# wenbowen123/iros20-6d-pose-tracking

Measured on AMD Instinct MI355X. Metric: RGB-D pair inferences/sec (176x176), higher is better.
Workload: dtype f32; 1 GPU; configs[1]: batch=64 synthetic 176x176 RGB-D pairs per GPU, random-init Se3TrackNet (reference state_dict surface), stage=full; pairs_per_gpu=64, global_batch=64, stage=full, frames=resident in HBM

## Files before the change

### iros20-6d-pose-tracking_amd/csrc/api.cpp

```cpp
#include <cmath>
#include <thread>
#include <cstdio>
#include <cstdlib>
#include <chrono>
#include <cstring>
#include <map>
#include <mutex>
#include <string>
#include <vector>

#include "se3tn_internal.h"
#include "weights.h"

using namespace se3tn;

static thread_local std::string g_err;
static int fail(int code, const std::string& msg) {
  g_err = msg;
  return code;
}
static int hipfail(hipError_t e, const char* what) {
  g_err = std::string(what) + ": " + hipGetErrorString(e);
  return (int)e;
}
// ... 7 lines not shown

struct GraphKey {
  const void *A, *B, *trans, *rot, *poseA, *poseB, *blob;
  int n, layout, prec, wino_min_batch, wino_tile, keep, wino64, wino64_fill;
  int small_kernels, splitk_fused, wino_fuse, gemmp, tail_parts;
  double tn, rn;
  bool operator==(const GraphKey& o) const { return std::memcmp(this, &o, sizeof(GraphKey)) == 0; }
};
struct GraphEntry {
  GraphKey key;
  hipGraphExec_t exec = nullptr;
  bool fast = false;
  const float* head_final = nullptr;
};

struct se3tn_ctx {
  int device = -1, max_batch = 0;
  TensorMap tensors;
  std::vector<float> packed;
  float* blob_owned = nullptr;
  const float* blob = nullptr;
  BlobLayout L;
  float *inA = nullptr, *inB = nullptr;
  float* stem = nullptr;
  float *pool = nullptr, *t64 = nullptr, *q64 = nullptr;
  float *ab = nullptr, *ab_t = nullptr;
  float *head = nullptr, *head_t = nullptr;
  float* head_f = nullptr;
  const float* head_final = nullptr;
  float* logits = nullptr;
  float* fcpart = nullptr;
  bool keep_intermediates = false;
  int auto_tile_override[2] = {0, 0};
  int trunk_kernel = 1;
  int gemmp = -1;
  bool wino_fuse = true;
  float* part = nullptr;
  int* splitk_sem = nullptr;
  int tail_parts_ch = 16;
  bool tail_parts = true;
  bool small_kernels = true;
  bool splitk_fused = false;
  size_t part_bytes = 0;
  int wino_min_batch = SE3TN_WINOGRAD_DEFAULT_MIN_BATCH;
  int wino_tile = SE3TN_WINOGRAD_DEFAULT_TILE;
  int wino_tile_derived = 0;
  float* wino_u[4] = {nullptr, nullptr, nullptr, nullptr};
  float* wino_u6[4] = {nullptr, nullptr, nullptr, nullptr};
  const float* wino6_blob = nullptr;
  float *wino_v = nullptr, *wino_m = nullptr;
  const float* wino_blob = nullptr;
  int wino64_min_batch = SE3TN_TRUNK_WINOGRAD_DEFAULT_MIN_BATCH;
  int wino64_min_fill = SE3TN_TRUNK_WINOGRAD_DEFAULT_MIN_FILL;
  int num_cus = 256;
  float* wino64_u[4] = {nullptr, nullptr, nullptr, nullptr};
  const float* wino64_blob = nullptr;
  SplitLayout SL;
  float* split_w = nullptr;
  const float* split_blob = nullptr;
  float* wino_us[4] = {nullptr, nullptr, nullptr, nullptr};
  float* wino_usc[4] = {nullptr, nullptr, nullptr, nullptr};
  const float* wino_us_blob = nullptr;
  int wino_us_tile = 0;
  int prec = SE3TN_PREC_F32;
  int offset_rule = SE3TN_OFFSET_RULE_NUMPY1;
  int raster_sub_bits = 4;
  uint8_t* trk_host = nullptr; uint8_t* trk_dev = nullptr; size_t trk_bytes = 0;
// ... 183 lines not shown
  c->fd_buf = nullptr; c->fd_pixels = 0;
  HIPCHK(hipMalloc((void**)&c->fd_buf, (3 * px + 2 + 4098 + 2) * sizeof(float)));
  c->fd_pixels = px;
  return SE3TN_OK;
}
static int reserve_zbuf(se3tn_ctx* c, size_t px) {
  if (px <= c->zbuf_px) return SE3TN_OK;
  HIPCHK(hipDeviceSynchronize());
  if (c->zbuf) HIPCHK(hipFree(c->zbuf));
  c->zbuf = nullptr; c->zbuf_px = 0;
  HIPCHK(hipMalloc((void**)&c->zbuf, sizeof(unsigned long long) * px));
  c->zbuf_px = px;
  return SE3TN_OK;
}
static bool stream_is_capturing(hipStream_t st) {
  hipStreamCaptureStatus cs = hipStreamCaptureStatusNone;
  return hipStreamIsCapturing(st, &cs) == hipSuccess && cs != hipStreamCaptureStatusNone;
}

extern "C" {

const char* se3tn_version(void) { return "se3tracknet-gfx950 0.5.0 (blob v7)"; }
const char* se3tn_last_error(void) { return g_err.c_str(); }

int se3tn_create(int device, int max_batch, se3tn_ctx** out) {
  if (!out || max_batch < 1) return fail(SE3TN_E_ARG, "se3tn_create: bad argument");
  se3tn_ctx* c = new se3tn_ctx();
  c->device = device;
  c->max_batch = max_batch;
  c->L = blob_layout();
  c->SL = split_layout();
  if (const char* e = std::getenv("SE3TN_WINOGRAD_AUTO_TILE_AB2")) c->auto_tile_override[0] = (std::atoi(e) == 4 || std::atoi(e) == 6) ? std::atoi(e) : 0;
  if (const char* e = std::getenv("SE3TN_WINOGRAD_AUTO_TILE_HEADS")) c->auto_tile_override[1] = (std::atoi(e) == 4 || std::atoi(e) == 6) ? std::atoi(e) : 0;
  if (const char* e = std::getenv("SE3TN_TRUNK_KERNEL")) c->trunk_kernel = std::atoi(e) == 2 ? 2 : 1;
  if (const char* e = std::getenv("SE3TN_WINO_GEMMP")) c->gemmp = std::atoi(e) != 0 ? 1 : 0;
  if (const char* e = std::getenv("SE3TN_WINOGRAD_FUSE")) c->wino_fuse = std::atoi(e) != 0;
  if (const char* e = std::getenv("SE3TN_TRUNK_WINOGRAD")) c->wino64_min_batch = std::atoi(e);
  if (const char* e = std::getenv("SE3TN_TRUNK_WINOGRAD_FILL")) c->wino64_min_fill = std::atoi(e);
  for (int i = 0; i < 8; ++i) { c->mean[i] = 0.0; c->stdv[i] = 1.0; }
  if (device >= 0) {
    hipDeviceProp_t prop;
    hipError_t e = hipGetDeviceProperties(&prop, device);
    if (e != hipSuccess) { delete c; return hipfail(e, "hipGetDeviceProperties"); }
    if (std::strncmp(prop.gcnArchName, "gfx950", 6) != 0) {
      std::string a = prop.gcnArchName;
      delete c;
      return fail(SE3TN_E_DEVICE, "device is " + a + ", this library is built for gfx950 only");
    }
    if (prop.multiProcessorCount > 0) c->num_cus = prop.multiProcessorCount;
    e = hipSetDevice(device);
    if (e != hipSuccess) { delete c; return hipfail(e, "hipSetDevice"); }
    const size_t mb = (size_t)max_batch;
    auto padded = [&](int s, int ch) { return (mb * (s + 2) * (s + 2) + PAD_SLACK_PX) * ch; };
    struct { float** p; size_t words; bool zero; } bufs[] = {
        {&c->inA, (mb * IN_P + IN_SLACK_ROWS) * IN_P * 4, true},
        {&c->inB, (mb * IN_P + IN_SLACK_ROWS) * IN_P * 4, true},
        {&c->stem, mb * S1 * S1 * 128, false}, {&c->pool, padded(S2, 128), true},
        {&c->t64, padded(S2, 128), true},      {&c->q64, padded(S2, 128), true},
        {&c->ab, padded(S3, 256), true},       {&c->ab_t, padded(S3, 256), true},
        {&c->head, padded(S4, 1024), true},    {&c->head_t, padded(S4, 1024), true},
        {&c->head_f, padded(S4, 1024), true},
        {&c->logits, mb * 6, true},           {&c->fcpart, mb * 192, true}};
    for (auto& b : bufs) {
      e = hipMalloc((void**)b.p, b.words * sizeof(float));
      if (e != hipSuccess) { se3tn_destroy(c); return hipfail(e, "hipMalloc(workspace)"); }
      if (b.zero) e = hipMemset(*b.p, 0, b.words * sizeof(float));
      if (e != hipSuccess) { se3tn_destroy(c); return hipfail(e, "hipMemset(workspace)"); }
// ... 1426 lines not shown
```

### iros20-6d-pose-tracking_amd/csrc/wino64_fused.hip

```cpp
#include "mfma_common.h"

#ifndef W64_KNOCKOUT
#define W64_KNOCKOUT 0
#endif

namespace se3tn {

namespace {
constexpr int W64_TILES = 11;
constexpr int W64_PATCH = 2 * W64_TILES + 2;
constexpr int W64_PATCH_FLOATS = W64_PATCH * W64_PATCH * 32;
constexpr int W64_V_FLOATS = 128 * 32, W64_U_FLOATS = 64 * 32;
constexpr int W64_UBUFS = 2;
constexpr int W64_LDS_FLOATS = W64_PATCH_FLOATS + 2 * W64_V_FLOATS + W64_UBUFS * W64_U_FLOATS;
constexpr int W64_YLDS_FLOATS = W64_TILES * W64_TILES * (4 * 64 + 4);
constexpr size_t W64_LDS_BYTES = sizeof(float) * (W64_YLDS_FLOATS > W64_LDS_FLOATS ? W64_YLDS_FLOATS : W64_LDS_FLOATS);
}

__device__ __forceinline__ void bt_row(int i, int& r0, int& r1, float& c0, float& c1) {
  r0 = i == 0 ? 0 : 1;
  r1 = i == 3 ? 3 : 2;
  c0 = i == 2 ? -1.f : 1.f;
  c1 = (i == 0 || i == 3) ? -1.f : 1.f;
}
__device__ __forceinline__ void at_col(int i, float& a0, float& a1) {
  a0 = i == 3 ? 0.f : 1.f;
  a1 = i == 0 ? 0.f : (i == 1 ? 1.f : -1.f);
}

template <bool NA, bool NB>
__device__ __forceinline__ float add_pm(const float a, const float b) {
  float r;
  if constexpr (!NA && !NB) asm volatile("v_add_f32 %0, %1, %2" : "=v"(r) : "v"(a), "v"(b));
  else if constexpr (NA && !NB) asm volatile("v_sub_f32 %0, %2, %1" : "=v"(r) : "v"(a), "v"(b));
  else if constexpr (!NA && NB) asm volatile("v_sub_f32 %0, %1, %2" : "=v"(r) : "v"(a), "v"(b));
  else asm volatile("v_sub_f32 %0, -%1, %2" : "=v"(r) : "v"(a), "v"(b));
  return r;
}
template <int K>
__device__ __forceinline__ void acc_pm(float& y, const float m) {
  if constexpr (K > 0) asm volatile("v_add_f32 %0, %0, %1" : "+v"(y) : "v"(m));
  else if constexpr (K < 0) asm volatile("v_sub_f32 %0, %0, %1" : "+v"(y) : "v"(m));
}
struct W64Tab {
  static constexpr int bt_r0(int i) { return i == 0 ? 0 : 1; }
  static constexpr int bt_r1(int i) { return i == 3 ? 3 : 2; }
  static constexpr bool bt_n0(int i) { return i == 2; }
  static constexpr bool bt_n1(int i) { return i == 0 || i == 3; }
  static constexpr int at(int y, int i) { return y == 0 ? (i == 3 ? 0 : 1) : (i == 0 ? 0 : (i == 1 ? 1 : -1)); }
  static constexpr int off(int r, int s) { return (r * W64_PATCH + (s >> 1) + 12 * (s & 1)) * 32; }
};

struct Wino64Args {
  const float* in;
  const float* U;
  const float* bias;
  const float* res;
  float* out;
  int in_ld, res_ld, out_ld;
  int in_gs, res_gs, out_gs, bias_gs;
  long long u_gs;
  int n, groups;
};

template <int EPI>
__global__ __launch_bounds__(512) void wino64_fused_kernel(const Wino64Args a) {
  extern __shared__ __attribute__((aligned(16))) float smem[];
  float* patch = smem;
  float* Vb = smem + W64_PATCH_FLOATS;
  float* Ub = Vb + 2 * W64_V_FLOATS;

  const int tid = threadIdx.x, lane = tid & 63;
  const int wid = __builtin_amdgcn_readfirstlane(tid >> 6);
  const int rb = wid >> 1, cbk = wid & 1;
  const int l31 = lane & 31, hh = lane >> 5;

  const int g = blockIdx.x % a.groups, rest = blockIdx.x / a.groups;
  const int quad = rest & 3, img = rest >> 2;
  const int y0 = (quad >> 1) * 2 * W64_TILES, x0 = (quad & 1) * 2 * W64_TILES;
  constexpr int HP = 46;
  const float* __restrict__ in = a.in + (size_t)g * a.in_gs + ((size_t)(img * HP + y0) * HP + x0) * a.in_ld;
  const float* __restrict__ Ug = a.U + (size_t)g * a.u_gs;
  const unsigned lds0 = __builtin_amdgcn_readfirstlane(lds_addr_of(smem));

  const int ur = tid >> 3;
  const unsigned uvoff = (unsigned)((ur * 32 + (((tid & 7) ^ ((ur >> 1) & 7)) << 2)) * 4);

#define W64_ISSUE_PATCH(CH)                                                                                     \
  {                                                                                                            \
    const float* pb_ = in + (CH) * 32;                                                                          \
    _Pragma("unroll") for (int j_ = 0; j_ < 9; ++j_) {                                \
      const int id_ = tid + 512 * j_, px_ = id_ >> 3, py_ = px_ / W64_PATCH, pxx_ = px_ - py_ * W64_PATCH;      \
      const int xs_ = pxx_ < 12 ? 2 * pxx_ : 2 * pxx_ - 23;           \
      glds16<0>(pb_, (unsigned)(((py_ * HP + xs_) * a.in_ld + (id_ & 7) * 4) * 4),                              \
                lds0 + (unsigned)((wid * 64 + 512 * j_) * 16));                                                 \
    }                                                                                                          \
  }
#define W64_ISSUE_U(CH, F, BUFI)                                                                                \
  glds16<0>(Ug + (size_t)((CH) * 16 + (F)) * W64_U_FLOATS, uvoff,                                              \
            lds0 + (unsigned)((W64_PATCH_FLOATS + 2 * W64_V_FLOATS + (BUFI) * W64_U_FLOATS + wid * 256) * 4));

  int tpix[2], tdst[2];
#pragma unroll
  for (int j = 0; j < 2; ++j) {
    const int tt = (tid + 512 * j) >> 3, tcb = tid & 7;
    const int ttr = tt < W64_TILES * W64_TILES ? tt : W64_TILES * W64_TILES - 1;
    const int tty = ttr / W64_TILES, ttx = ttr - tty * W64_TILES;
    tpix[j] = ((2 * tty) * W64_PATCH + ttx) * 32 + tcb * 4;
    tdst[j] = tt * 32 + ((tcb ^ ((tt >> 1) & 7)) << 2);
  }
#define W64_BT(F)                                                                                               \
  int r0_, r1_, s0_, s1_;                                                                                      \
  float cr0_, cr1_, cs0_, cs1_;                                                                                \
  bt_row((F) >> 2, r0_, r1_, cr0_, cr1_);                                                                      \
  bt_row((F) & 3, s0_, s1_, cs0_, cs1_);                                                                       \
  const int q0_ = (s0_ >> 1) + 12 * (s0_ & 1), q1_ = (s1_ >> 1) + 12 * (s1_ & 1);              \
  const int o00_ = (r0_ * W64_PATCH + q0_) * 32, o01_ = (r0_ * W64_PATCH + q1_) * 32;                          \
  const int o10_ = (r1_ * W64_PATCH + q0_) * 32, o11_ = (r1_ * W64_PATCH + q1_) * 32;                          \
  const float c00_ = cr0_ * cs0_, c01_ = cr0_ * cs1_, c10_ = cr1_ * cs0_, c11_ = cr1_ * cs1_;
#define W64_TR_LOAD(D)                                                                                          \
  _Pragma("unroll") for (int j_ = 0; j_ < 2; ++j_) {                                                            \
    D[j_][0] = *reinterpret_cast<const float4*>(patch + tpix[j_] + o00_);                                       \
    D[j_][1] = *reinterpret_cast<const float4*>(patch + tpix[j_] + o01_);                                       \
    D[j_][2] = *reinterpret_cast<const float4*>(patch + tpix[j_] + o10_);                                       \
    D[j_][3] = *reinterpret_cast<const float4*>(patch + tpix[j_] + o11_);                                       \
  }
#define W64_TR_STORE(D, VBUF)                                                                                   \
  _Pragma("unroll") for (int j_ = 0; j_ < 2; ++j_) {                                                            \
    float4 v_;                                                                                                 \
    v_.x = c00_ * D[j_][0].x + c01_ * D[j_][1].x + c10_ * D[j_][2].x + c11_ * D[j_][3].x;                       \
    v_.y = c00_ * D[j_][0].y + c01_ * D[j_][1].y + c10_ * D[j_][2].y + c11_ * D[j_][3].y;                       \
    v_.z = c00_ * D[j_][0].z + c01_ * D[j_][1].z + c10_ * D[j_][2].z + c11_ * D[j_][3].z;                       \
    v_.w = c00_ * D[j_][0].w + c01_ * D[j_][1].w + c10_ * D[j_][2].w + c11_ * D[j_][3].w;                       \
    *reinterpret_cast<float4*>(Vb + (VBUF) * W64_V_FLOATS + tdst[j_]) = v_;                                     \
  }
#define W64_TRANSFORM(F, VBUF)                                                                                  \
  {                                                                                                            \
    W64_BT(F)                                                                                                  \
    float4 d_[2][4];                                                                                           \
    W64_TR_LOAD(d_)                                                                                            \
    W64_TR_STORE(d_, VBUF)                                                                                     \
  }

  const int X = (l31 >> 1) & 7;
  const int lo = (hh ^ (X & 1)) * 4, xk = X >> 1;
  const int fo0 = ((0 ^ xk) << 3) + lo, fo1 = ((1 ^ xk) << 3) + lo, fo2 = ((2 ^ xk) << 3) + lo, fo3 = ((3 ^ xk) << 3) + lo;

  float Y[16][4];
#pragma unroll
  for (int e = 0; e < 16; ++e)
#pragma unroll
    for (int o = 0; o < 4; ++o) Y[e][o] = 0.f;

  W64_ISSUE_PATCH(0)
  W64_ISSUE_U(0, 0, 0)
  wait_dma_and_barrier();
  W64_TRANSFORM(0, 0)
  __syncthreads();

  f32x16 accA, accB;
#pragma unroll
  for (int e = 0; e < 16; ++e) accB[e] = 0.f;
  const f32x16 zero16 = {0.f, 0.f, 0.f, 0.f, 0.f, 0.f, 0.f, 0.f, 0.f, 0.f, 0.f, 0.f, 0.f, 0.f, 0.f, 0.f};
#define W64_FOLD(PREV, F)                                                                                       \
  {                                                                                                            \
    float ay0_, ay1_, ax0_, ax1_;                                                                              \
    at_col((F) >> 2, ay0_, ay1_);                                                                              \
    at_col((F) & 3, ax0_, ax1_);                                                                               \
    const float k00_ = ay0_ * ax0_, k01_ = ay0_ * ax1_, k10_ = ay1_ * ax0_, k11_ = ay1_ * ax1_;                \
    _Pragma("unroll") for (int e_ = 0; e_ < 16; ++e_) {                                                        \
      const float m_ = PREV[e_];                                                                               \
      Y[e_][0] += k00_ * m_; Y[e_][1] += k01_ * m_; Y[e_][2] += k10_ * m_; Y[e_][3] += k11_ * m_;              \
    }                                                                                                          \
  }
#define W64_MFMA(ACC)                                                                                        \
  ACC = q_ == 0 ? __builtin_amdgcn_mfma_f32_32x32x2f32(wv_[0], pv_[0], zero16, 0, 0, 0)                         \
                : __builtin_amdgcn_mfma_f32_32x32x2f32(wv_[q_], pv_[q_], ACC, 0, 0, 0);
#define W64_STEP(F, ACC, PREV)                                                                                  \
  {                                                                                                            \
    constexpr int f_ = (F), buf = f_ & 1, fn_ = (f_ + 1) & 15, fp_ = (f_ + 15) & 15;                            \
    const bool last_ = ch == 1 && f_ == 15;                                                                    \
    if (!last_) W64_ISSUE_U(f_ == 15 ? 1 : ch, fn_, buf ^ 1)                                                    \
    if (f_ == 15 && ch == 0) W64_ISSUE_PATCH(1)  \
    {                                                                                                          \
      const float* pP = Vb + buf * W64_V_FLOATS + (rb * 32 + l31) * 32;                                        \
      const float* pW = Ub + buf * W64_U_FLOATS + (cbk * 32 + l31) * 32;                                       \
      float pv_[16], wv_[16];                                                                                  \
      float d_[2][4][4], v_[2][4];                                       \
      *reinterpret_cast<float4*>(pv_ + 0) = *reinterpret_cast<const float4*>(pP + fo0);                         \
      *reinterpret_cast<float4*>(wv_ + 0) = *reinterpret_cast<const float4*>(pW + fo0);                         \
      *reinterpret_cast<float4*>(pv_ + 4) = *reinterpret_cast<const float4*>(pP + fo1);                         \
      *reinterpret_cast<float4*>(wv_ + 4) = *reinterpret_cast<const float4*>(pW + fo1);                         \
      *reinterpret_cast<float4*>(pv_ + 8) = *reinterpret_cast<const float4*>(pP + fo2);                         \
      *reinterpret_cast<float4*>(wv_ + 8) = *reinterpret_cast<const float4*>(pW + fo2);                         \
      *reinterpret_cast<float4*>(pv_ + 12) = *reinterpret_cast<const float4*>(pP + fo3);                        \
      *reinterpret_cast<float4*>(wv_ + 12) = *reinterpret_cast<const float4*>(pW + fo3);                        \
                              \
       \
      constexpr int i_ = fn_ >> 2, j_ = fn_ & 3;                                                               \
      constexpr int oo_[4] = {W64Tab::off(W64Tab::bt_r0(i_), W64Tab::bt_r0(j_)), W64Tab::off(W64Tab::bt_r0(i_), W64Tab::bt_r1(j_)), \
                              W64Tab::off(W64Tab::bt_r1(i_), W64Tab::bt_r0(j_)), W64Tab::off(W64Tab::bt_r1(i_), W64Tab::bt_r1(j_))}; \
      constexpr bool nn_[4] = {W64Tab::bt_n0(i_) != W64Tab::bt_n0(j_), W64Tab::bt_n0(i_) != W64Tab::bt_n1(j_),  \
                               W64Tab::bt_n1(i_) != W64Tab::bt_n0(j_), W64Tab::bt_n1(i_) != W64Tab::bt_n1(j_)}; \
      _Pragma("unroll") for (int t_ = 0; t_ < 2; ++t_)                                                          \
        _Pragma("unroll") for (int w_ = 0; w_ < 4; ++w_) {                                                      \
          if (W64_KNOCKOUT & 1) *reinterpret_cast<float4*>(d_[t_][w_]) = make_float4(1.f, 2.f, 3.f, 4.f);  \
          else *reinterpret_cast<float4*>(d_[t_][w_]) = *reinterpret_cast<const float4*>(patch + tpix[t_] + oo_[w_]); \
        }                                                                                                      \
      constexpr int pi_ = fp_ >> 2, pj_ = fp_ & 3;    \
      __builtin_amdgcn_sched_barrier(0);                                                                       \
      _Pragma("unroll") for (int q_ = 0; q_ < 16; ++q_) {                                                       \
        W64_MFMA(ACC)                                                                                          \
        __builtin_amdgcn_sched_barrier(0);                                                                     \
        if (q_ < 8) {                             \
          _Pragma("unroll") for (int e_ = 2 * q_; e_ < 2 * q_ + 2; ++e_) {                                      \
            const float m_ = PREV[e_];                                                                         \
            acc_pm<W64Tab::at(0, pi_) * W64Tab::at(0, pj_)>(Y[e_][0], m_);                                     \
            acc_pm<W64Tab::at(0, pi_) * W64Tab::at(1, pj_)>(Y[e_][1], m_);                                     \
            acc_pm<W64Tab::at(1, pi_) * W64Tab::at(0, pj_)>(Y[e_][2], m_);                                     \
            acc_pm<W64Tab::at(1, pi_) * W64Tab::at(1, pj_)>(Y[e_][3], m_);                                     \
          }                                                                                                    \
        } else {               \
          const int t_ = (q_ - 8) >> 2, x_ = (q_ - 8) & 3;                                                     \
          v_[t_][x_] = add_pm<false, false>(add_pm<nn_[0], nn_[1]>(d_[t_][0][x_], d_[t_][1][x_]),              \
                                            add_pm<nn_[2], nn_[3]>(d_[t_][2][x_], d_[t_][3][x_]));             \
        }                                                                                                      \
        __builtin_amdgcn_sched_barrier(0);                                                                     \
      }                                                                                                        \
      *reinterpret_cast<float4*>(Vb + (buf ^ 1) * W64_V_FLOATS + tdst[0]) = *reinterpret_cast<float4*>(v_[0]); \
      *reinterpret_cast<float4*>(Vb + (buf ^ 1) * W64_V_FLOATS + tdst[1]) = *reinterpret_cast<float4*>(v_[1]); \
    }                                                                                                          \
    if (!last_) wait_dma_and_barrier();                                                                        \
    if (f_ == 15 && ch == 0) {  \
      W64_TRANSFORM(0, 0)                                                                                      \
      __syncthreads();                                                                                         \
    }                                                                                                          \
  }
  for (int ch = 0; ch < 2; ++ch) {
    W64_STEP(0, accA, accB) W64_STEP(1, accB, accA) W64_STEP(2, accA, accB) W64_STEP(3, accB, accA)
    W64_STEP(4, accA, accB) W64_STEP(5, accB, accA) W64_STEP(6, accA, accB) W64_STEP(7, accB, accA)
    W64_STEP(8, accA, accB) W64_STEP(9, accB, accA) W64_STEP(10, accA, accB) W64_STEP(11, accB, accA)
    W64_STEP(12, accA, accB) W64_STEP(13, accB, accA) W64_STEP(14, accA, accB) W64_STEP(15, accB, accA)
  }
  W64_FOLD(accB, 15)
#undef W64_STEP
#undef W64_MFMA
#undef W64_FOLD
#undef W64_ISSUE_PATCH
#undef W64_ISSUE_U
#undef W64_TRANSFORM
#undef W64_TR_LOAD
#undef W64_TR_STORE
#undef W64_BT

  constexpr int YS = 4 * 64 + 4;
  __syncthreads();
  {
    const int t = rb * 32 + l31;
    if (t < W64_TILES * W64_TILES) {
#pragma unroll
      for (int o = 0; o < 4; ++o)
#pragma unroll
        for (int q = 0; q < 4; ++q)
          *reinterpret_cast<float4*>(smem + t * YS + o * 64 + cbk * 32 + q * 8 + hh * 4) =
              make_float4(Y[4 * q + 0][o], Y[4 * q + 1][o], Y[4 * q + 2][o], Y[4 * q + 3][o]);
    }
  }
  const float* __restrict__ bias = a.bias + (size_t)g * a.bias_gs;
  const float* __restrict__ res = (EPI == 1) ? a.res + (size_t)g * a.res_gs : nullptr;
  float* __restrict__ out = a.out + (size_t)g * a.out_gs;
  const int c4 = (tid & 15) * 4;
  __syncthreads();
  const float4 b = *reinterpret_cast<const float4*>(bias + c4);
#pragma unroll 4
  for (int k = 0; k < 16; ++k) {
    const int p = (k * 512 + tid) >> 4;
    const int t = p >> 2, o = p & 3;
    if (t < W64_TILES * W64_TILES) {
      const int ty = t / W64_TILES, tx = t - ty * W64_TILES;
      const int oy = y0 + 2 * ty + (o >> 1) + 1, ox = x0 + 2 * tx + (o & 1) + 1;
      const size_t pix = (size_t)(img * HP + oy) * HP + ox;
      float4 v = *reinterpret_cast<const float4*>(smem + t * YS + o * 64 + c4);
      v.x += b.x; v.y += b.y; v.z += b.z; v.w += b.w;
      if (EPI == 1) {
        const float4 r = *reinterpret_cast<const float4*>(res + pix * a.res_ld + c4);
        v.x += r.x; v.y += r.y; v.z += r.z; v.w += r.w;
      }
      v.x = fmaxf(v.x, 0.f); v.y = fmaxf(v.y, 0.f); v.z = fmaxf(v.z, 0.f); v.w = fmaxf(v.w, 0.f);
      *reinterpret_cast<float4*>(out + pix * a.out_ld + c4) = v;
    }
  }
}

#ifndef SE3TN_TRUNK_REGV
#define SE3TN_TRUNK_REGV 0
#endif
#if SE3TN_TRUNK_REGV
typedef float f32x4 __attribute__((ext_vector_type(4)));

template <int EPI>
__global__ __launch_bounds__(512) void wino64_regv_kernel(const Wino64Args a) {
  extern __shared__ __attribute__((aligned(16))) float smem[];
  const int tid = threadIdx.x, lane = tid & 63;
  const int wid = __builtin_amdgcn_readfirstlane(tid >> 6);
  const int r16 = lane & 15, jq = lane >> 4;

  const int g = blockIdx.x % a.groups, rest = blockIdx.x / a.groups;
  const int quad = rest & 3, img = rest >> 2;
  const int y0 = (quad >> 1) * 2 * W64_TILES, x0 = (quad & 1) * 2 * W64_TILES;
  constexpr int HP = 46;
  const float* __restrict__ in = a.in + (size_t)g * a.in_gs + ((size_t)(img * HP + y0) * HP + x0) * a.in_ld;
  const float* __restrict__ Ug = a.U + (size_t)g * a.u_gs;
  const unsigned lds0 = __builtin_amdgcn_readfirstlane(lds_addr_of(smem));

#define W64R_ISSUE_PATCH(CH)                                                                                    \
  {                                                                                                            \
    const float* pb_ = in + (CH) * 32;                                                                          \
    _Pragma("unroll") for (int j_ = 0; j_ < 9; ++j_) {                                                          \
      const int id_ = tid + 512 * j_, px_ = id_ >> 3, py_ = px_ / W64_PATCH, lc_ = px_ - py_ * W64_PATCH;       \
      const int xs_ = lc_ < 12 ? 2 * lc_ : 2 * lc_ - 23;                                                        \
      glds16<0>(pb_, (unsigned)(((py_ * HP + xs_) * a.in_ld + (((id_ & 7) ^ (lc_ & 7)) << 2)) * 4),             \
                lds0 + (unsigned)(((CH) * W64_PATCH_FLOATS) * 4 + (wid * 64 + 512 * j_) * 16));                 \
    }                                                                                                          \
  }
// ... 126 lines not shown
  const float4 bq = *reinterpret_cast<const float4*>(bias + c4);
#pragma unroll 4
  for (int k = 0; k < 16; ++k) {
    const int p = (k * 512 + tid) >> 4;
    const int t = p >> 2, o = p & 3;
    if (t < W64_TILES * W64_TILES) {
      const int ty = t / W64_TILES, tx = t - ty * W64_TILES;
      const int oy = y0 + 2 * ty + (o >> 1) + 1, ox = x0 + 2 * tx + (o & 1) + 1;
      const size_t pix = (size_t)(img * HP + oy) * HP + ox;
      float4 v = *reinterpret_cast<const float4*>(smem + t * YS + o * 64 + c4);
      v.x += bq.x; v.y += bq.y; v.z += bq.z; v.w += bq.w;
      if (EPI == 1) {
        const float4 r = *reinterpret_cast<const float4*>(res + pix * a.res_ld + c4);
        v.x += r.x; v.y += r.y; v.z += r.z; v.w += r.w;
      }
      v.x = fmaxf(v.x, 0.f); v.y = fmaxf(v.y, 0.f); v.z = fmaxf(v.z, 0.f); v.w = fmaxf(v.w, 0.f);
      *reinterpret_cast<float4*>(out + pix * a.out_ld + c4) = v;
    }
  }
}

#endif

hipError_t launch_wino64(const float* in, int in_ld, int in_gs, const float* U, long long u_gs, const float* bias, int bias_gs,
                         const float* res, int res_ld, int res_gs, float* out, int out_ld, int out_gs, int n, int groups, int epi,
                         int variant, hipStream_t st) {
  Wino64Args a{};
  a.in = in; a.U = U; a.bias = bias; a.res = res; a.out = out;
  a.in_ld = in_ld; a.res_ld = res_ld; a.out_ld = out_ld;
  a.in_gs = in_gs; a.res_gs = res_gs; a.out_gs = out_gs; a.bias_gs = bias_gs; a.u_gs = u_gs;
  a.n = n; a.groups = groups;
  constexpr size_t lds2 = sizeof(float) * 2 * W64_PATCH_FLOATS;
  static_assert(lds2 >= sizeof(float) * W64_YLDS_FLOATS, "the epilogue staging must fit the patch buffers");
  static PerDeviceOnce attr[4];
#if !SE3TN_TRUNK_REGV
  variant = 1;
#endif
  const void* kern = epi == 1 ? reinterpret_cast<const void*>(wino64_fused_kernel<1>) : reinterpret_cast<const void*>(wino64_fused_kernel<0>);
#if SE3TN_TRUNK_REGV
  if (variant == 2) kern = epi == 1 ? reinterpret_cast<const void*>(wino64_regv_kernel<1>) : reinterpret_cast<const void*>(wino64_regv_kernel<0>);
#endif
  const size_t lds = variant == 2 ? lds2 : W64_LDS_BYTES;
  bool* done = attr[(variant == 2 ? 2 : 0) + (epi == 1 ? 1 : 0)].current();
  if (!done || !*done) {
    hipError_t e = hipFuncSetAttribute(kern, hipFuncAttributeMaxDynamicSharedMemorySize, (int)lds);
    if (e != hipSuccess) return e;
    if (done) *done = true;
  }
  const dim3 grid(n * 4 * groups);
#if SE3TN_TRUNK_REGV
  if (variant == 2) {
    if (epi == 1) hipLaunchKernelGGL(wino64_regv_kernel<1>, grid, dim3(512), lds, st, a);
    else hipLaunchKernelGGL(wino64_regv_kernel<0>, grid, dim3(512), lds, st, a);
    return hipGetLastError();
  }
#endif
  if (epi == 1) hipLaunchKernelGGL(wino64_fused_kernel<1>, grid, dim3(512), lds, st, a);
  else hipLaunchKernelGGL(wino64_fused_kernel<0>, grid, dim3(512), lds, st, a);
  return hipGetLastError();
}

}
```

Measured before the change: 41960 pairs/s.

## Split trunk Winograd patch loads into half-row chunks interleaved across filter steps

Result: no change. 42170 pairs/s, median of 6 (+0.5%).

```diff
diff --git a/iros20-6d-pose-tracking_amd/csrc/api.cpp b/iros20-6d-pose-tracking_amd/csrc/api.cpp
--- a/iros20-6d-pose-tracking_amd/csrc/api.cpp
+++ b/iros20-6d-pose-tracking_amd/csrc/api.cpp
@@ -63,7 +63,7 @@
   float* fcpart = nullptr;
   bool keep_intermediates = false;
   int auto_tile_override[2] = {0, 0};
-  int trunk_kernel = 1;
+  int trunk_kernel = 3;
   int gemmp = -1;
   bool wino_fuse = true;
   float* part = nullptr;
@@ -313,7 +313,7 @@
   c->SL = split_layout();
   if (const char* e = std::getenv("SE3TN_WINOGRAD_AUTO_TILE_AB2")) c->auto_tile_override[0] = (std::atoi(e) == 4 || std::atoi(e) == 6) ? std::atoi(e) : 0;
   if (const char* e = std::getenv("SE3TN_WINOGRAD_AUTO_TILE_HEADS")) c->auto_tile_override[1] = (std::atoi(e) == 4 || std::atoi(e) == 6) ? std::atoi(e) : 0;
-  if (const char* e = std::getenv("SE3TN_TRUNK_KERNEL")) c->trunk_kernel = std::atoi(e) == 2 ? 2 : 1;
+  if (const char* e = std::getenv("SE3TN_TRUNK_KERNEL")) c->trunk_kernel = (std::atoi(e) == 1 || std::atoi(e) == 2) ? std::atoi(e) : 3;
   if (const char* e = std::getenv("SE3TN_WINO_GEMMP")) c->gemmp = std::atoi(e) != 0 ? 1 : 0;
   if (const char* e = std::getenv("SE3TN_WINOGRAD_FUSE")) c->wino_fuse = std::atoi(e) != 0;
   if (const char* e = std::getenv("SE3TN_TRUNK_WINOGRAD")) c->wino64_min_batch = std::atoi(e);
diff --git a/iros20-6d-pose-tracking_amd/csrc/wino64_fused.hip b/iros20-6d-pose-tracking_amd/csrc/wino64_fused.hip
--- a/iros20-6d-pose-tracking_amd/csrc/wino64_fused.hip
+++ b/iros20-6d-pose-tracking_amd/csrc/wino64_fused.hip
@@ -2,6 +2,29 @@
 
 #ifndef W64_KNOCKOUT
 #define W64_KNOCKOUT 0
+#endif
+
+#ifdef SE3TN_W64_TRACE
+#define W64_TRACE_SLOTS 104
+__device__ unsigned long long se3tn_w64_trace[4 * 2 * 8 * W64_TRACE_SLOTS];
+extern "C" int se3tn_debug_w64_trace(void* host_out, size_t bytes, int clear) {
+  if (clear) {
+    void* p = nullptr;
+    if (hipGetSymbolAddress(&p, HIP_SYMBOL(se3tn_w64_trace)) != hipSuccess) return 1;
+    return (int)hipMemset(p, 0, sizeof(se3tn_w64_trace));
+  }
+  return (int)hipMemcpyFromSymbol(host_out, HIP_SYMBOL(se3tn_w64_trace), bytes, 0, hipMemcpyDeviceToHost);
+}
+#define W64_TRACE_SETUP                                                                                          \
+  const bool tr_on_ = lane == 0 && (blockIdx.x == 0 || blockIdx.x == gridDim.x - 1);                              \
+  unsigned long long* tr_ = ::se3tn_w64_trace +                                                                  \
+      ((((a.groups == 2 ? 0 : 2) + EPI) * 2 + (blockIdx.x == 0 ? 0 : 1)) * 8 + wid) * W64_TRACE_SLOTS;
+#define W64_STAMP(I) if (tr_on_) tr_[(I)] = __builtin_amdgcn_s_memtime();
+#define W64_STAMP_RT(I) if (tr_on_) tr_[(I)] = __builtin_amdgcn_s_memrealtime();
+#else
+#define W64_TRACE_SETUP
+#define W64_STAMP(I)
+#define W64_STAMP_RT(I)
 #endif
 
 namespace se3tn {
@@ -63,7 +86,15 @@
   int n, groups;
 };
 
-template <int EPI>
+__device__ __forceinline__ void wait_vm_and_barrier(const int n) {
+  if (n == 0) asm volatile("s_waitcnt vmcnt(0)" ::: "memory");
+  else if (n == 1) asm volatile("s_waitcnt vmcnt(1)" ::: "memory");
+  else if (n == 2) asm volatile("s_waitcnt vmcnt(2)" ::: "memory");
+  else asm volatile("s_waitcnt vmcnt(3)" ::: "memory");
+  __syncthreads();
+}
+
+template <int EPI, bool SPLIT>
 __global__ __launch_bounds__(512) void wino64_fused_kernel(const Wino64Args a) {
   extern __shared__ __attribute__((aligned(16))) float smem[];
   float* patch = smem;
@@ -72,6 +103,9 @@
 
   const int tid = threadIdx.x, lane = tid & 63;
   const int wid = __builtin_amdgcn_readfirstlane(tid >> 6);
+  W64_TRACE_SETUP
+  W64_STAMP_RT(101)
+  W64_STAMP(0)
   const int rb = wid >> 1, cbk = wid & 1;
   const int l31 = lane & 31, hh = lane >> 5;
 
@@ -99,6 +133,16 @@
 #define W64_ISSUE_U(CH, F, BUFI)                                                                                \
   glds16<0>(Ug + (size_t)((CH) * 16 + (F)) * W64_U_FLOATS, uvoff,                                              \
             lds0 + (unsigned)((W64_PATCH_FLOATS + 2 * W64_V_FLOATS + (BUFI) * W64_U_FLOATS + wid * 256) * 4));
+#define W64_ISSUE_HALF(CH, P, J)                                                                                \
+  {                                                                                                            \
+    const int q_ = wid + 8 * (J), hr_ = q_ / 3, py_ = 2 * hr_ + (P), lc0_ = (q_ - 3 * hr_) * 8;                 \
+    const int lc_ = lc0_ + (lane >> 3), xs_ = lc_ < 12 ? 2 * lc_ : 2 * lc_ - 23;                                \
+    glds16<0>(in + (CH) * 32, (unsigned)(((py_ * HP + xs_) * a.in_ld + (lane & 7) * 4) * 4),                    \
+              lds0 + (unsigned)((py_ * W64_PATCH + lc0_) * 32 * 4));                                            \
+  }
+#define W64_ISSUE_HALF_A(CH, P) { W64_ISSUE_HALF(CH, P, 0) W64_ISSUE_HALF(CH, P, 1) if (wid < 4) W64_ISSUE_HALF(CH, P, 4) }
+#define W64_ISSUE_HALF_B(CH, P) { W64_ISSUE_HALF(CH, P, 2) W64_ISSUE_HALF(CH, P, 3) }
+  const int vm_a = wid < 4 ? 3 : 2, vm_b = 2;
 
   int tpix[2], tdst[2];
 #pragma unroll
@@ -152,11 +196,18 @@
 #pragma unroll
     for (int o = 0; o < 4; ++o) Y[e][o] = 0.f;
 
-  W64_ISSUE_PATCH(0)
+  if constexpr (SPLIT) {
+    W64_ISSUE_HALF_A(0, 0)
+    W64_ISSUE_HALF_B(0, 0)
+  } else {
+    W64_ISSUE_PATCH(0)
+  }
   W64_ISSUE_U(0, 0, 0)
   wait_dma_and_barrier();
+  W64_STAMP(1)
   W64_TRANSFORM(0, 0)
   __syncthreads();
+  W64_STAMP(2)
 
   f32x16 accA, accB;
 #pragma unroll
@@ -180,8 +231,17 @@
   {                                                                                                            \
     constexpr int f_ = (F), buf = f_ & 1, fn_ = (f_ + 1) & 15, fp_ = (f_ + 15) & 15;                            \
     const bool last_ = ch == 1 && f_ == 15;                                                                    \
+    W64_STAMP(3 + 3 * (16 * ch + f_))                                                                          \
     if (!last_) W64_ISSUE_U(f_ == 15 ? 1 : ch, fn_, buf ^ 1)                                                    \
-    if (f_ == 15 && ch == 0) W64_ISSUE_PATCH(1)  \
+    int vm_ = 0;    \
+    if constexpr (SPLIT) {                                                                                     \
+      if (f_ == 0 && ch == 0) { W64_ISSUE_HALF_A(0, 1) vm_ = vm_a; }                                           \
+      if (f_ == 1 && ch == 0) { W64_ISSUE_HALF_B(0, 1) vm_ = vm_b; }                                           \
+      if (f_ == 11 && ch == 0) { W64_ISSUE_HALF_A(1, 0) vm_ = vm_a; }   \
+      if (f_ == 12 && ch == 0) { W64_ISSUE_HALF_B(1, 0) vm_ = vm_b; }                                          \
+      if (f_ == 15 && ch == 0) { W64_ISSUE_HALF_A(1, 1) vm_ = vm_a; }   \
+      if (f_ == 0 && ch == 1) { W64_ISSUE_HALF_B(1, 1) vm_ = vm_b; }                                           \
+    } else if (f_ == 15 && ch == 0) W64_ISSUE_PATCH(1)  \
     {                                                                                                          \
       const float* pP = Vb + buf * W64_V_FLOATS + (rb * 32 + l31) * 32;                                        \
       const float* pW = Ub + buf * W64_U_FLOATS + (cbk * 32 + l31) * 32;                                       \
@@ -222,18 +282,28 @@
           }                                                                                                    \
         } else {               \
           const int t_ = (q_ - 8) >> 2, x_ = (q_ - 8) & 3;                                                     \
-          v_[t_][x_] = add_pm<false, false>(add_pm<nn_[0], nn_[1]>(d_[t_][0][x_], d_[t_][1][x_]),              \
-                                            add_pm<nn_[2], nn_[3]>(d_[t_][2][x_], d_[t_][3][x_]));             \
+          if constexpr (SPLIT && fn_ == 0)  \
+            v_[t_][x_] = add_pm<false, nn_[3]>(add_pm<false, nn_[2]>(add_pm<nn_[0], nn_[1]>(d_[t_][0][x_], d_[t_][1][x_]), \
+                                                                     d_[t_][2][x_]), d_[t_][3][x_]);           \
+          else                                                                                                 \
+            v_[t_][x_] = add_pm<false, false>(add_pm<nn_[0], nn_[1]>(d_[t_][0][x_], d_[t_][1][x_]),            \
+                                              add_pm<nn_[2], nn_[3]>(d_[t_][2][x_], d_[t_][3][x_]));           \
         }                                                                                                      \
         __builtin_amdgcn_sched_barrier(0);                                                                     \
       }                                                                                                        \
       *reinterpret_cast<float4*>(Vb + (buf ^ 1) * W64_V_FLOATS + tdst[0]) = *reinterpret_cast<float4*>(v_[0]); \
       *reinterpret_cast<float4*>(Vb + (buf ^ 1) * W64_V_FLOATS + tdst[1]) = *reinterpret_cast<float4*>(v_[1]); \
     }                                                                                                          \
-    if (!last_) wait_dma_and_barrier();                                                                        \
-    if (f_ == 15 && ch == 0) {  \
+    W64_STAMP(4 + 3 * (16 * ch + f_))                                                                          \
+    if (!last_) {                                                                                              \
+      if constexpr (SPLIT) wait_vm_and_barrier(vm_);  \
+      else wait_dma_and_barrier();                                                                             \
+    }                                                                                                          \
+    W64_STAMP(5 + 3 * (16 * ch + f_))                                                                          \
+    if (!SPLIT && f_ == 15 && ch == 0) {  \
       W64_TRANSFORM(0, 0)                                                                                      \
       __syncthreads();                                                                                         \
+      W64_STAMP(103)                                                                                           \
     }                                                                                                          \
   }
   for (int ch = 0; ch < 2; ++ch) {
@@ -243,11 +313,15 @@
     W64_STEP(12, accA, accB) W64_STEP(13, accB, accA) W64_STEP(14, accA, accB) W64_STEP(15, accB, accA)
   }
   W64_FOLD(accB, 15)
+  W64_STAMP(99)
 #undef W64_STEP
 #undef W64_MFMA
 #undef W64_FOLD
 #undef W64_ISSUE_PATCH
 #undef W64_ISSUE_U
+#undef W64_ISSUE_HALF
+#undef W64_ISSUE_HALF_A
+#undef W64_ISSUE_HALF_B
 #undef W64_TRANSFORM
 #undef W64_TR_LOAD
 #undef W64_TR_STORE
@@ -290,6 +364,8 @@
       *reinterpret_cast<float4*>(out + pix * a.out_ld + c4) = v;
     }
   }
+  W64_STAMP(100)
+  W64_STAMP_RT(102)
 }
 
 #ifndef SE3TN_TRUNK_REGV
@@ -482,16 +558,20 @@
   a.n = n; a.groups = groups;
   constexpr size_t lds2 = sizeof(float) * 2 * W64_PATCH_FLOATS;
   static_assert(lds2 >= sizeof(float) * W64_YLDS_FLOATS, "the epilogue staging must fit the patch buffers");
-  static PerDeviceOnce attr[4];
+  static PerDeviceOnce attr[6];
 #if !SE3TN_TRUNK_REGV
-  variant = 1;
-#endif
-  const void* kern = epi == 1 ? reinterpret_cast<const void*>(wino64_fused_kernel<1>) : reinterpret_cast<const void*>(wino64_fused_kernel<0>);
+  if (variant == 2) variant = 3;
+#endif
+  if (variant != 1 && variant != 2) variant = 3;
+  const void* kern = variant == 1 ? (epi == 1 ? reinterpret_cast<const void*>(wino64_fused_kernel<1, false>)
+                                              : reinterpret_cast<const void*>(wino64_fused_kernel<0, false>))
+                                  : (epi == 1 ? reinterpret_cast<const void*>(wino64_fused_kernel<1, true>)
+                                              : reinterpret_cast<const void*>(wino64_fused_kernel<0, true>));
 #if SE3TN_TRUNK_REGV
   if (variant == 2) kern = epi == 1 ? reinterpret_cast<const void*>(wino64_regv_kernel<1>) : reinterpret_cast<const void*>(wino64_regv_kernel<0>);
 #endif
   const size_t lds = variant == 2 ? lds2 : W64_LDS_BYTES;
-  bool* done = attr[(variant == 2 ? 2 : 0) + (epi == 1 ? 1 : 0)].current();
+  bool* done = attr[2 * (variant - 1) + (epi == 1 ? 1 : 0)].current();
   if (!done || !*done) {
     hipError_t e = hipFuncSetAttribute(kern, hipFuncAttributeMaxDynamicSharedMemorySize, (int)lds);
     if (e != hipSuccess) return e;
@@ -505,8 +585,13 @@
     return hipGetLastError();
   }
 #endif
-  if (epi == 1) hipLaunchKernelGGL(wino64_fused_kernel<1>, grid, dim3(512), lds, st, a);
-  else hipLaunchKernelGGL(wino64_fused_kernel<0>, grid, dim3(512), lds, st, a);
+  if (variant == 1) {
+    if (epi == 1) hipLaunchKernelGGL((wino64_fused_kernel<1, false>), grid, dim3(512), lds, st, a);
+    else hipLaunchKernelGGL((wino64_fused_kernel<0, false>), grid, dim3(512), lds, st, a);
+  } else {
+    if (epi == 1) hipLaunchKernelGGL((wino64_fused_kernel<1, true>), grid, dim3(512), lds, st, a);
+    else hipLaunchKernelGGL((wino64_fused_kernel<0, true>), grid, dim3(512), lds, st, a);
+  }
   return hipGetLastError();
 }
 
```

## Reorder Winograd frequencies to accumulate corner terms in MFMA and reuse BT partials

Applied to the files above, without the earlier changes.

Result: no change. 42040 pairs/s before, 42370 pairs/s after, median of 6 (+0.8%).

```diff
diff --git a/iros20-6d-pose-tracking_amd/csrc/wino64_fused.hip b/iros20-6d-pose-tracking_amd/csrc/wino64_fused.hip
--- a/iros20-6d-pose-tracking_amd/csrc/wino64_fused.hip
+++ b/iros20-6d-pose-tracking_amd/csrc/wino64_fused.hip
@@ -17,17 +17,6 @@
 constexpr size_t W64_LDS_BYTES = sizeof(float) * (W64_YLDS_FLOATS > W64_LDS_FLOATS ? W64_YLDS_FLOATS : W64_LDS_FLOATS);
 }
 
-__device__ __forceinline__ void bt_row(int i, int& r0, int& r1, float& c0, float& c1) {
-  r0 = i == 0 ? 0 : 1;
-  r1 = i == 3 ? 3 : 2;
-  c0 = i == 2 ? -1.f : 1.f;
-  c1 = (i == 0 || i == 3) ? -1.f : 1.f;
-}
-__device__ __forceinline__ void at_col(int i, float& a0, float& a1) {
-  a0 = i == 3 ? 0.f : 1.f;
-  a1 = i == 0 ? 0.f : (i == 1 ? 1.f : -1.f);
-}
-
 template <bool NA, bool NB>
 __device__ __forceinline__ float add_pm(const float a, const float b) {
   float r;
@@ -42,6 +31,14 @@
   if constexpr (K > 0) asm volatile("v_add_f32 %0, %0, %1" : "+v"(y) : "v"(m));
   else if constexpr (K < 0) asm volatile("v_sub_f32 %0, %0, %1" : "+v"(y) : "v"(m));
 }
+template <int K>
+__device__ __forceinline__ void acc_pm(f32x16& y, const int e, const float m) {
+  if constexpr (K != 0) {
+    float t = y[e];
+    acc_pm<K>(t, m);
+    y[e] = t;
+  }
+}
 struct W64Tab {
   static constexpr int bt_r0(int i) { return i == 0 ? 0 : 1; }
   static constexpr int bt_r1(int i) { return i == 3 ? 3 : 2; }
@@ -49,6 +46,16 @@
   static constexpr bool bt_n1(int i) { return i == 0 || i == 3; }
   static constexpr int at(int y, int i) { return y == 0 ? (i == 3 ? 0 : 1) : (i == 0 ? 0 : (i == 1 ? 1 : -1)); }
   static constexpr int off(int r, int s) { return (r * W64_PATCH + (s >> 1) + 12 * (s & 1)) * 32; }
+  static constexpr int order(int p) { return p < 4 ? (p == 0 ? 0 : p == 1 ? 3 : p - 1) : p < 8 ? 12 + order(p - 4) : p - 4; }
+  static constexpr bool corner(int f) { return ((f >> 2) == 0 || (f >> 2) == 3) && ((f & 3) == 0 || (f & 3) == 3); }
+  static constexpr int target(int f) { return 2 * ((f >> 2) == 3) + ((f & 3) == 3); }
+  static constexpr int foldk(int f, int o) {
+    return corner(f) ? 0 : at(o >> 1, f >> 2) * at(o & 1, f & 3) * ((o == 1 || o == 2) ? -1 : 1);
+  }
+  static constexpr bool fresh(int f, int s) {
+    return s == 0 || s == 3 || (s == 2 && (f & 3) == 0) ||
+           (s == 1 && ((f & 3) == ((f >> 2) == 0 || (f >> 2) == 3 ? 3 : 1)));
+  }
 };
 
 struct Wino64Args {
@@ -109,79 +116,54 @@
     tpix[j] = ((2 * tty) * W64_PATCH + ttx) * 32 + tcb * 4;
     tdst[j] = tt * 32 + ((tcb ^ ((tt >> 1) & 7)) << 2);
   }
-#define W64_BT(F)                                                                                               \
-  int r0_, r1_, s0_, s1_;                                                                                      \
-  float cr0_, cr1_, cs0_, cs1_;                                                                                \
-  bt_row((F) >> 2, r0_, r1_, cr0_, cr1_);                                                                      \
-  bt_row((F) & 3, s0_, s1_, cs0_, cs1_);                                                                       \
-  const int q0_ = (s0_ >> 1) + 12 * (s0_ & 1), q1_ = (s1_ >> 1) + 12 * (s1_ & 1);              \
-  const int o00_ = (r0_ * W64_PATCH + q0_) * 32, o01_ = (r0_ * W64_PATCH + q1_) * 32;                          \
-  const int o10_ = (r1_ * W64_PATCH + q0_) * 32, o11_ = (r1_ * W64_PATCH + q1_) * 32;                          \
-  const float c00_ = cr0_ * cs0_, c01_ = cr0_ * cs1_, c10_ = cr1_ * cs0_, c11_ = cr1_ * cs1_;
-#define W64_TR_LOAD(D)                                                                                          \
-  _Pragma("unroll") for (int j_ = 0; j_ < 2; ++j_) {                                                            \
-    D[j_][0] = *reinterpret_cast<const float4*>(patch + tpix[j_] + o00_);                                       \
-    D[j_][1] = *reinterpret_cast<const float4*>(patch + tpix[j_] + o01_);                                       \
-    D[j_][2] = *reinterpret_cast<const float4*>(patch + tpix[j_] + o10_);                                       \
-    D[j_][3] = *reinterpret_cast<const float4*>(patch + tpix[j_] + o11_);                                       \
-  }
-#define W64_TR_STORE(D, VBUF)                                                                                   \
-  _Pragma("unroll") for (int j_ = 0; j_ < 2; ++j_) {                                                            \
-    float4 v_;                                                                                                 \
-    v_.x = c00_ * D[j_][0].x + c01_ * D[j_][1].x + c10_ * D[j_][2].x + c11_ * D[j_][3].x;                       \
-    v_.y = c00_ * D[j_][0].y + c01_ * D[j_][1].y + c10_ * D[j_][2].y + c11_ * D[j_][3].y;                       \
-    v_.z = c00_ * D[j_][0].z + c01_ * D[j_][1].z + c10_ * D[j_][2].z + c11_ * D[j_][3].z;                       \
-    v_.w = c00_ * D[j_][0].w + c01_ * D[j_][1].w + c10_ * D[j_][2].w + c11_ * D[j_][3].w;                       \
-    *reinterpret_cast<float4*>(Vb + (VBUF) * W64_V_FLOATS + tdst[j_]) = v_;                                     \
-  }
-#define W64_TRANSFORM(F, VBUF)                                                                                  \
+  float R1[2][4], R2[2][4];
+#define W64_TRANSFORM0()                                                                                        \
   {                                                                                                            \
-    W64_BT(F)                                                                                                  \
-    float4 d_[2][4];                                                                                           \
-    W64_TR_LOAD(d_)                                                                                            \
-    W64_TR_STORE(d_, VBUF)                                                                                     \
+    constexpr int oo_[4] = {W64Tab::off(0, 0), W64Tab::off(2, 0), W64Tab::off(0, 2), W64Tab::off(2, 2)};       \
+    float d_[2][4][4], v_[2][4];                                                                               \
+    _Pragma("unroll") for (int t_ = 0; t_ < 2; ++t_)                                                            \
+      _Pragma("unroll") for (int w_ = 0; w_ < 4; ++w_)                                                          \
+        *reinterpret_cast<float4*>(d_[t_][w_]) = *reinterpret_cast<const float4*>(patch + tpix[t_] + oo_[w_]);  \
+    _Pragma("unroll") for (int t_ = 0; t_ < 2; ++t_)                                                            \
+      _Pragma("unroll") for (int x_ = 0; x_ < 4; ++x_) {                                                        \
+        R2[t_][x_] = add_pm<false, true>(d_[t_][2][x_], d_[t_][3][x_]);                                         \
+        v_[t_][x_] = add_pm<false, true>(add_pm<false, true>(d_[t_][0][x_], d_[t_][1][x_]), R2[t_][x_]);        \
+      }                                                                                                        \
+    *reinterpret_cast<float4*>(Vb + tdst[0]) = *reinterpret_cast<float4*>(v_[0]);                               \
+    *reinterpret_cast<float4*>(Vb + tdst[1]) = *reinterpret_cast<float4*>(v_[1]);                               \
   }
 
   const int X = (l31 >> 1) & 7;
   const int lo = (hh ^ (X & 1)) * 4, xk = X >> 1;
   const int fo0 = ((0 ^ xk) << 3) + lo, fo1 = ((1 ^ xk) << 3) + lo, fo2 = ((2 ^ xk) << 3) + lo, fo3 = ((3 ^ xk) << 3) + lo;
 
-  float Y[16][4];
-#pragma unroll
-  for (int e = 0; e < 16; ++e)
-#pragma unroll
-    for (int o = 0; o < 4; ++o) Y[e][o] = 0.f;
+  f32x16 Yv[4];
+#pragma unroll
+  for (int o = 0; o < 4; ++o)
+#pragma unroll
+    for (int e = 0; e < 16; ++e) Yv[o][e] = 0.f;
 
   W64_ISSUE_PATCH(0)
-  W64_ISSUE_U(0, 0, 0)
+  W64_ISSUE_U(0, W64Tab::order(0), 0)
   wait_dma_and_barrier();
-  W64_TRANSFORM(0, 0)
+  W64_TRANSFORM0()
   __syncthreads();
 
   f32x16 accA, accB;
 #pragma unroll
   for (int e = 0; e < 16; ++e) accB[e] = 0.f;
   const f32x16 zero16 = {0.f, 0.f, 0.f, 0.f, 0.f, 0.f, 0.f, 0.f, 0.f, 0.f, 0.f, 0.f, 0.f, 0.f, 0.f, 0.f};
-#define W64_FOLD(PREV, F)                                                                                       \
+#define W64_MFMA(ACC)                                                                                           \
+  if constexpr (W64Tab::corner(f_)) ACC = __builtin_amdgcn_mfma_f32_32x32x2f32(wv_[q_], pv_[q_], ACC, 0, 0, 0);  \
+  else ACC = q_ == 0 ? __builtin_amdgcn_mfma_f32_32x32x2f32(wv_[0], pv_[0], zero16, 0, 0, 0)                      \
+                     : __builtin_amdgcn_mfma_f32_32x32x2f32(wv_[q_], pv_[q_], ACC, 0, 0, 0);
+#define W64_STEP(P, ACC, PREV)                                                                                  \
   {                                                                                                            \
-    float ay0_, ay1_, ax0_, ax1_;                                                                              \
-    at_col((F) >> 2, ay0_, ay1_);                                                                              \
-    at_col((F) & 3, ax0_, ax1_);                                                                               \
-    const float k00_ = ay0_ * ax0_, k01_ = ay0_ * ax1_, k10_ = ay1_ * ax0_, k11_ = ay1_ * ax1_;                \
-    _Pragma("unroll") for (int e_ = 0; e_ < 16; ++e_) {                                                        \
-      const float m_ = PREV[e_];                                                                               \
-      Y[e_][0] += k00_ * m_; Y[e_][1] += k01_ * m_; Y[e_][2] += k10_ * m_; Y[e_][3] += k11_ * m_;              \
-    }                                                                                                          \
-  }
-#define W64_MFMA(ACC)                                                                                        \
-  ACC = q_ == 0 ? __builtin_amdgcn_mfma_f32_32x32x2f32(wv_[0], pv_[0], zero16, 0, 0, 0)                         \
-                : __builtin_amdgcn_mfma_f32_32x32x2f32(wv_[q_], pv_[q_], ACC, 0, 0, 0);
-#define W64_STEP(F, ACC, PREV)                                                                                  \
-  {                                                                                                            \
-    constexpr int f_ = (F), buf = f_ & 1, fn_ = (f_ + 1) & 15, fp_ = (f_ + 15) & 15;                            \
-    const bool last_ = ch == 1 && f_ == 15;                                                                    \
-    if (!last_) W64_ISSUE_U(f_ == 15 ? 1 : ch, fn_, buf ^ 1)                                                    \
-    if (f_ == 15 && ch == 0) W64_ISSUE_PATCH(1)  \
+    constexpr int p_ = (P), buf = p_ & 1;                                                                      \
+    constexpr int f_ = W64Tab::order(p_), fn_ = W64Tab::order((p_ + 1) & 15), fp_ = W64Tab::order((p_ + 15) & 15); \
+    const bool last_ = ch == 1 && p_ == 15;                                                                    \
+    if (!last_) W64_ISSUE_U(p_ == 15 ? 1 : ch, fn_, buf ^ 1)                                                    \
+    if (p_ == 15 && ch == 0) W64_ISSUE_PATCH(1)  \
     {                                                                                                          \
       const float* pP = Vb + buf * W64_V_FLOATS + (rb * 32 + l31) * 32;                                        \
       const float* pW = Ub + buf * W64_U_FLOATS + (cbk * 32 + l31) * 32;                                       \
@@ -195,35 +177,46 @@
       *reinterpret_cast<float4*>(wv_ + 8) = *reinterpret_cast<const float4*>(pW + fo2);                         \
       *reinterpret_cast<float4*>(pv_ + 12) = *reinterpret_cast<const float4*>(pP + fo3);                        \
       *reinterpret_cast<float4*>(wv_ + 12) = *reinterpret_cast<const float4*>(pW + fo3);                        \
-                              \
        \
-      constexpr int i_ = fn_ >> 2, j_ = fn_ & 3;                                                               \
-      constexpr int oo_[4] = {W64Tab::off(W64Tab::bt_r0(i_), W64Tab::bt_r0(j_)), W64Tab::off(W64Tab::bt_r0(i_), W64Tab::bt_r1(j_)), \
-                              W64Tab::off(W64Tab::bt_r1(i_), W64Tab::bt_r0(j_)), W64Tab::off(W64Tab::bt_r1(i_), W64Tab::bt_r1(j_))}; \
-      constexpr bool nn_[4] = {W64Tab::bt_n0(i_) != W64Tab::bt_n0(j_), W64Tab::bt_n0(i_) != W64Tab::bt_n1(j_),  \
-                               W64Tab::bt_n1(i_) != W64Tab::bt_n0(j_), W64Tab::bt_n1(i_) != W64Tab::bt_n1(j_)}; \
+       \
+       \
+      constexpr int i_ = fn_ >> 2, j_ = fn_ & 3, s0_ = W64Tab::bt_r0(j_), s1_ = W64Tab::bt_r1(j_);              \
+      constexpr bool new0_ = W64Tab::fresh(fn_, s0_), new1_ = W64Tab::fresh(fn_, s1_);                         \
+      constexpr bool ni0_ = W64Tab::bt_n0(i_), ni1_ = W64Tab::bt_n1(i_), nj0_ = W64Tab::bt_n0(j_), nj1_ = W64Tab::bt_n1(j_); \
+      constexpr int oo_[4] = {W64Tab::off(W64Tab::bt_r0(i_), s0_), W64Tab::off(W64Tab::bt_r1(i_), s0_),         \
+                              W64Tab::off(W64Tab::bt_r0(i_), s1_), W64Tab::off(W64Tab::bt_r1(i_), s1_)};        \
       _Pragma("unroll") for (int t_ = 0; t_ < 2; ++t_)                                                          \
         _Pragma("unroll") for (int w_ = 0; w_ < 4; ++w_) {                                                      \
+          if (w_ < 2 ? !new0_ : !new1_) continue;                                                              \
           if (W64_KNOCKOUT & 1) *reinterpret_cast<float4*>(d_[t_][w_]) = make_float4(1.f, 2.f, 3.f, 4.f);  \
           else *reinterpret_cast<float4*>(d_[t_][w_]) = *reinterpret_cast<const float4*>(patch + tpix[t_] + oo_[w_]); \
         }                                                                                                      \
-      constexpr int pi_ = fp_ >> 2, pj_ = fp_ & 3;    \
       __builtin_amdgcn_sched_barrier(0);                                                                       \
       _Pragma("unroll") for (int q_ = 0; q_ < 16; ++q_) {                                                       \
         W64_MFMA(ACC)                                                                                          \
         __builtin_amdgcn_sched_barrier(0);                                                                     \
-        if (q_ < 8) {                             \
+        if (q_ < 8) {        \
           _Pragma("unroll") for (int e_ = 2 * q_; e_ < 2 * q_ + 2; ++e_) {                                      \
             const float m_ = PREV[e_];                                                                         \
-            acc_pm<W64Tab::at(0, pi_) * W64Tab::at(0, pj_)>(Y[e_][0], m_);                                     \
-            acc_pm<W64Tab::at(0, pi_) * W64Tab::at(1, pj_)>(Y[e_][1], m_);                                     \
-            acc_pm<W64Tab::at(1, pi_) * W64Tab::at(0, pj_)>(Y[e_][2], m_);                                     \
-            acc_pm<W64Tab::at(1, pi_) * W64Tab::at(1, pj_)>(Y[e_][3], m_);                                     \
+            acc_pm<W64Tab::foldk(fp_, 0)>(Yv[0], e_, m_);                                                      \
+            acc_pm<W64Tab::foldk(fp_, 1)>(Yv[1], e_, m_);                                                      \
+            acc_pm<W64Tab::foldk(fp_, 2)>(Yv[2], e_, m_);                                                      \
+            acc_pm<W64Tab::foldk(fp_, 3)>(Yv[3], e_, m_);                                                      \
           }                                                                                                    \
         } else {               \
           const int t_ = (q_ - 8) >> 2, x_ = (q_ - 8) & 3;                                                     \
-          v_[t_][x_] = add_pm<false, false>(add_pm<nn_[0], nn_[1]>(d_[t_][0][x_], d_[t_][1][x_]),              \
-                                            add_pm<nn_[2], nn_[3]>(d_[t_][2][x_], d_[t_][3][x_]));             \
+          float a_, b_;                                                                                        \
+          if constexpr (s0_ == 0) a_ = add_pm<ni0_, ni1_>(d_[t_][0][x_], d_[t_][1][x_]);                       \
+          else {                                                                                               \
+            if constexpr (new0_) R1[t_][x_] = add_pm<ni0_, ni1_>(d_[t_][0][x_], d_[t_][1][x_]);                \
+            a_ = R1[t_][x_];                                                                                   \
+          }                                                                                                    \
+          if constexpr (s1_ == 3) b_ = add_pm<ni0_, ni1_>(d_[t_][2][x_], d_[t_][3][x_]);                       \
+          else {                                                                                               \
+            if constexpr (new1_) R2[t_][x_] = add_pm<ni0_, ni1_>(d_[t_][2][x_], d_[t_][3][x_]);                \
+            b_ = R2[t_][x_];                                                                                   \
+          }                                                                                                    \
+          v_[t_][x_] = add_pm<nj0_, nj1_>(a_, b_);                                                             \
         }                                                                                                      \
         __builtin_amdgcn_sched_barrier(0);                                                                     \
       }                                                                                                        \
@@ -231,27 +224,38 @@
       *reinterpret_cast<float4*>(Vb + (buf ^ 1) * W64_V_FLOATS + tdst[1]) = *reinterpret_cast<float4*>(v_[1]); \
     }                                                                                                          \
     if (!last_) wait_dma_and_barrier();                                                                        \
-    if (f_ == 15 && ch == 0) {  \
-      W64_TRANSFORM(0, 0)                                                                                      \
+    if (p_ == 15 && ch == 0) {  \
+      W64_TRANSFORM0()                                                                                         \
       __syncthreads();                                                                                         \
     }                                                                                                          \
   }
+  static_assert(W64Tab::target(W64Tab::order(0)) == 0 && W64Tab::target(W64Tab::order(1)) == 1 &&
+                    W64Tab::target(W64Tab::order(4)) == 2 && W64Tab::target(W64Tab::order(5)) == 3 &&
+                    W64Tab::corner(W64Tab::order(0)) && W64Tab::corner(W64Tab::order(1)) && W64Tab::corner(W64Tab::order(4)) &&
+                    W64Tab::corner(W64Tab::order(5)) && !W64Tab::corner(W64Tab::order(2)) && !W64Tab::corner(W64Tab::order(6)),
+                "the accumulator arguments of W64_STEP follow W64Tab::order");
   for (int ch = 0; ch < 2; ++ch) {
-    W64_STEP(0, accA, accB) W64_STEP(1, accB, accA) W64_STEP(2, accA, accB) W64_STEP(3, accB, accA)
-    W64_STEP(4, accA, accB) W64_STEP(5, accB, accA) W64_STEP(6, accA, accB) W64_STEP(7, accB, accA)
+    W64_STEP(0, Yv[0], accB) W64_STEP(1, Yv[1], accA) W64_STEP(2, accA, accB) W64_STEP(3, accB, accA)
+    W64_STEP(4, Yv[2], accB) W64_STEP(5, Yv[3], accA) W64_STEP(6, accA, accB) W64_STEP(7, accB, accA)
     W64_STEP(8, accA, accB) W64_STEP(9, accB, accA) W64_STEP(10, accA, accB) W64_STEP(11, accB, accA)
     W64_STEP(12, accA, accB) W64_STEP(13, accB, accA) W64_STEP(14, accA, accB) W64_STEP(15, accB, accA)
   }
-  W64_FOLD(accB, 15)
+  {
+    constexpr int fp_ = W64Tab::order(15), k0 = W64Tab::foldk(fp_, 0), k1 = W64Tab::foldk(fp_, 1), k2 = W64Tab::foldk(fp_, 2),
+                  k3 = W64Tab::foldk(fp_, 3);
+#pragma unroll
+    for (int e = 0; e < 16; ++e) {
+      if (k0 != 0) Yv[0][e] += (float)k0 * accB[e];
+      if (k1 != 0) Yv[1][e] += (float)k1 * accB[e];
+      if (k2 != 0) Yv[2][e] += (float)k2 * accB[e];
+      if (k3 != 0) Yv[3][e] += (float)k3 * accB[e];
+    }
+  }
 #undef W64_STEP
 #undef W64_MFMA
-#undef W64_FOLD
 #undef W64_ISSUE_PATCH
 #undef W64_ISSUE_U
-#undef W64_TRANSFORM
-#undef W64_TR_LOAD
-#undef W64_TR_STORE
-#undef W64_BT
+#undef W64_TRANSFORM0
 
   constexpr int YS = 4 * 64 + 4;
   __syncthreads();
@@ -259,11 +263,13 @@
     const int t = rb * 32 + l31;
     if (t < W64_TILES * W64_TILES) {
 #pragma unroll
-      for (int o = 0; o < 4; ++o)
+      for (int o = 0; o < 4; ++o) {
+        const float sg = (o == 1 || o == 2) ? -1.f : 1.f;
 #pragma unroll
         for (int q = 0; q < 4; ++q)
           *reinterpret_cast<float4*>(smem + t * YS + o * 64 + cbk * 32 + q * 8 + hh * 4) =
-              make_float4(Y[4 * q + 0][o], Y[4 * q + 1][o], Y[4 * q + 2][o], Y[4 * q + 3][o]);
+              make_float4(sg * Yv[o][4 * q + 0], sg * Yv[o][4 * q + 1], sg * Yv[o][4 * q + 2], sg * Yv[o][4 * q + 3]);
+      }
     }
   }
   const float* __restrict__ bias = a.bias + (size_t)g * a.bias_gs;
```
